# mitschabaude/msm-zprize

Measured on AMD Instinct MI355X. Metric: Mpoint-adds/s (ms per MSM in ms_per_step), higher is better.
Workload: dtype u32 limbs (28-bit lazy Montgomery, i64 accumulate)

## Files before the change

msm_zprize_amd/_native.py:

```python
import ctypes as C
import os

HERE = os.path.dirname(os.path.abspath(__file__))
LIB_PATH = os.environ.get("MSMZ_LIB") or os.path.join(HERE, "libmsmz.so")

MSMZ_N_STAGES = 8
STAGE_NAMES = ["digits", "scan", "scatter", "plan", "accumulate", "reduce", "final", "total"]


class MsmzOpts(C.Structure):
    _fields_ = [("c", C.c_int32), ("glv", C.c_int32), ("safe", C.c_int32), ("buckets", C.c_int32),
                ("timing", C.c_int32), ("reserved", C.c_int32 * 3)]


class MsmzLog(C.Structure):
    _fields_ = [("stage_ms", C.c_float * MSMZ_N_STAGES), ("c", C.c_int32), ("K", C.c_int32), ("rounds", C.c_int32),
                ("glv", C.c_int32), ("n_entries", C.c_uint64), ("n_pairs", C.c_uint64), ("max_bucket", C.c_uint32),
                ("scatter_launches", C.c_uint32), ("scatter_kernel_ms", C.c_float), ("batch_add_ms", C.c_float * 32)]


MSMZ_SRC_DEVICE, MSMZ_SRC_MONTGOMERY, MSMZ_SRC_DEFAULT_STREAM = 1, 2, 4
MSMZ_SRC_COMPRESSED, MSMZ_SRC_SIGN_PARITY = 8, 16
MSMZ_ERR_POINT = 7

# ... 170 lines not shown
    "msmz_scalars_sumcheck_round": (C.c_int, [C.c_void_p, C.POINTER(MsmzSumcheck), C.POINTER(C.c_uint32), C.c_char_p]),
    "msmz_point_add": (C.c_int, [C.c_int, C.c_char_p, C.c_int, C.c_char_p, C.c_int, C.c_char_p, C.POINTER(C.c_int)]),
    "msmz_test_set_glv_bits": (C.c_int, [C.c_void_p, C.c_int]),
    "msmz_test_retries": (C.c_int, [C.c_void_p]),
    "msmz_test_set_limits": (C.c_int, [C.c_void_p, C.c_uint64, C.c_uint64]),
    "msmz_test_passes": (C.c_int, [C.c_void_p, C.POINTER(C.c_uint64), C.POINTER(C.c_uint64)]),
    "msmz_test_scalar_dot_geometry": (None, [C.POINTER(C.c_uint32), C.POINTER(C.c_uint32)]),
    "msmz_test_scalar_scan_geometry": (None, [C.POINTER(C.c_uint32), C.POINTER(C.c_uint32), C.POINTER(C.c_uint32)]),
    "msmz_test_ntt_plan": (C.c_int, [C.c_int, C.c_uint32, C.POINTER(C.c_uint32), C.POINTER(C.c_uint32)]),
    "msmz_test_ntt_geometry": (None, [C.POINTER(C.c_uint32)]),
    "msmz_test_mle_geometry": (None, [C.POINTER(C.c_uint32), C.POINTER(C.c_uint32), C.POINTER(C.c_uint32)]),
    "msmz_test_fixed_base_plan": (C.c_int, [C.c_int, C.c_uint64, C.c_int, C.POINTER(C.c_int32), C.POINTER(C.c_int32),
                                            C.POINTER(C.c_uint64)]),
    "msmz_test_set_fixed_base_window": (C.c_int, [C.c_void_p, C.c_int]),
    "msmz_test_fixed_base_tables": (C.c_int, [C.c_void_p, C.POINTER(C.c_uint64)]),
    "msmz_test_field": (C.c_int, [C.c_void_p, C.c_int, C.c_char_p, C.c_char_p, C.c_uint64, C.c_char_p]),
    "msmz_test_field_limbs": (C.c_int, [C.c_void_p, C.c_int, C.c_void_p, C.c_void_p, C.c_uint64, C.c_void_p,
                                        C.c_char_p]),
    "msmz_test_field_rows": (C.c_int, [C.c_void_p, C.c_int, C.c_void_p, C.c_void_p, C.c_uint64, C.c_uint32, C.c_void_p,
                                       C.c_char_p]),
    "msmz_test_glv": (C.c_int, [C.c_void_p, C.c_char_p, C.c_uint64, C.c_char_p, C.c_char_p, C.c_char_p]),
    "msmz_test_digits": (C.c_int, [C.c_void_p, C.c_char_p, C.c_uint64, C.c_int, C.c_int, C.c_int, C.c_void_p]),
    "msmz_test_sort": (C.c_int, [C.c_void_p, C.c_char_p, C.c_uint64, C.c_int, C.c_int, C.c_int, C.c_void_p, C.c_void_p,
                                 C.c_uint64, C.c_void_p, C.c_uint64]),
    "msmz_test_sort_ex": (C.c_int, [C.c_void_p, C.POINTER(MsmzTestSortArgs)]),
    "msmz_test_point_raw": (C.c_int, [C.c_void_p, C.c_int, C.c_char_p, C.c_char_p, C.c_char_p, C.c_uint64, C.c_int,
                                      C.c_char_p]),
    "msmz_test_point": (C.c_int, [C.c_void_p, C.c_int, C.c_char_p, C.c_char_p, C.c_char_p, C.c_char_p, C.c_uint64,
                                  C.c_char_p]),
    "msmz_test_batch_add": (C.c_int, [C.c_void_p, C.c_int, C.c_int, C.c_char_p, C.c_char_p, C.c_uint64, C.c_char_p,
                                      C.c_char_p, C.c_uint64, C.c_void_p, C.c_uint64, C.c_uint64, C.c_char_p,
                                      C.POINTER(C.c_uint32)]),
    "msmz_test_reduce": (C.c_int, [C.c_void_p, C.POINTER(MsmzTestReduceArgs)]),
    "msmz_test_plan": (C.c_int, [C.c_void_p, C.POINTER(MsmzTestPlanArgs)]),
}

_lib = None


class MsmzError(RuntimeError):
    def __init__(self, status, where):
        self.status = status
        msg = lib().msmz_strerror(status).decode() if _lib is not None else "?"
        super().__init__(f"{where}: msmz status {status} ({msg})")


def lib():
    global _lib
    if _lib is None:
        if not os.path.exists(LIB_PATH):
            raise RuntimeError(f"{LIB_PATH} is missing: run `python -m msm_zprize_amd.build` "
                               "(the MSM has no CPU fallback)")
        l = C.CDLL(LIB_PATH)
        for name, (res, args) in EXPORTS.items():
            fn = getattr(l, name)
            fn.restype = res
            fn.argtypes = args
        _lib = l
    return _lib


def check(status, where):
    if status != 0:
        raise MsmzError(status, where)
```

msm_zprize_amd/csrc/instantiate.h:

```cpp
#pragma once
#include "check_kernels.h"
#include "export_kernels.h"
#include "fixed_kernels.h"
#include "gen_kernels.h"
#include "import_kernels.h"
#include "kernels.h"
#include "mle_kernels.h"
#include "mul_kernels.h"
#include "ntt_kernels.h"
#include "scalar_kernels.h"
#include "scan_kernels.h"
#include "test_kernels.h"

#if !defined(MSMZ_CURVE) || MSMZ_CURVE == 0
#define MSMZ_W0(X) X(Bls377Fp, Bls377Fr)
#else
#define MSMZ_W0(X)
#endif
#if !defined(MSMZ_CURVE) || MSMZ_CURVE == 1
#define MSMZ_W1(X) X(PallasFp, PallasFr)
#else
#define MSMZ_W1(X)
#endif
#if !defined(MSMZ_CURVE) || MSMZ_CURVE == 2
// ... 15 lines not shown
#ifndef MSMZ_BATCH_OCC
#define MSMZ_BATCH_OCC 4
#endif
#ifndef MSMZ_BATCH_BMAX
#define MSMZ_BATCH_BMAX 16
#endif

#define MSMZ_INST_BATCH(F, Fr, PFX)                                                                               \
  PFX template __global__ void k_batch_add<F, MSMZ_BATCH_T, true, MSMZ_BATCH_OCC, MSMZ_BATCH_BMAX>(              \
      uint32_t*, const uint32_t*, const uint2*, uint32_t, uint32_t, int, MsmMeta*);                              \
  PFX template __global__ void k_batch_add<F, MSMZ_BATCH_T, false, MSMZ_BATCH_OCC, MSMZ_BATCH_BMAX>(             \
      uint32_t*, const uint32_t*, const uint2*, uint32_t, uint32_t, int, MsmMeta*);

#define MSMZ_INST_POLICY(P, PFX)                                                                                 \
  PFX template __global__ void k_reduce_quad<P>(uint32_t*, uint32_t*, const uint32_t*, const uint32_t*, uint32_t, \
                                                uint32_t, uint32_t);                                             \
  PFX template __global__ void k_reduce_quad16<P>(uint32_t*, uint32_t*, const uint32_t*, const uint32_t*,        \
                                                  uint32_t, uint32_t, uint32_t);                                 \
  PFX template __global__ void k_reduce_tail<P>(uint32_t*, uint32_t*, uint32_t*, uint32_t*, uint32_t*, uint32_t, \
                                                uint32_t);                                                       \
  PFX template __global__ void k_reduce_rows<P>(uint32_t*, uint32_t*, const uint32_t*, const uint32_t*, uint32_t, \
                                                uint32_t, uint32_t);                                             \
  PFX template __global__ void k_pairsum<P>(uint32_t*, const uint32_t*, uint32_t);                               \
  PFX template __global__ void k_fill_neutral<P>(uint32_t*, uint32_t);                                           \
  PFX template __global__ void k_bucket_sums<P>(uint32_t*, const uint32_t*, const uint32_t*, uint32_t);          \
  PFX template __global__ void k_reduce2d_partial_acc<P>(uint32_t*, const uint32_t*, const uint32_t*, R2Geom, uint32_t); \
  PFX template __global__ void k_pairsum_x4<P>(uint32_t*, const uint32_t*, uint32_t);                            \
  PFX template __global__ void k_bucket_accumulate<P>(uint32_t*, const uint32_t*, const uint32_t*,               \
                                                      const uint32_t*, const uint32_t*, uint32_t, uint32_t, int);

#define MSMZ_INST_REDUCE(F, Fr, PFX)                                                                              \
  PFX template __global__ void k_reduce2d_partial<F>(uint32_t*, const uint32_t*, const uint32_t*, const uint4*,   \
                                                     R2Geom, uint32_t);                                          \
  PFX template __global__ void k_reduce_affine_finish<F>(uint32_t*, uint32_t*, const uint32_t*, const uint32_t*,  \
                                                         const uint2*, const uint4*, F2Geom);                     \
  MSMZ_INST_POLICY(WeierPolicy<F>, PFX)

#define MSMZ_INST_REDUCE_TE(F, Fr, PFX) MSMZ_INST_POLICY(TePolicy<F>, PFX)

#define MSMZ_INST_TEST(F, Fr, P, PFX)                                                                             \
  PFX template __global__ void k_test_field<F>(uint32_t*, const uint32_t*, const uint32_t*, uint32_t, int, uint32_t*); \
  PFX template __global__ void k_test_field_limbs<F>(int32_t*, uint32_t*, const int32_t*, const int32_t*, uint32_t,  \
                                                      int, uint32_t*);                                            \
  PFX template __global__ void k_test_field_rows<F>(int32_t*, uint32_t*, const int32_t*, const int32_t*, uint32_t,   \
                                                     int, uint32_t);                                              \
  PFX template __global__ void k_test_glv<Fr>(uint32_t*, uint32_t*, uint8_t*, const uint32_t*, uint32_t);         \
  PFX template __global__ void k_test_digits<Fr, false>(uint32_t*, const uint32_t*, uint32_t, int, int);          \
  PFX template __global__ void k_test_point<P>(uint32_t*, const uint32_t*, const uint32_t*, const uint8_t*,   \
                                                   const uint8_t*, uint32_t, int);                                \
  PFX template __global__ void k_test_point_raw<P>(uint32_t*, const uint32_t*, const uint32_t*, const uint8_t*, \
                                                       uint32_t, int, int);                                       \
  PFX template __global__ void k_test_accs_in<P>(uint32_t*, const uint32_t*, const uint8_t*, const uint32_t*, \
                                                     uint32_t, uint32_t*);                                        \
  PFX template __global__ void k_test_accs_out<P>(uint32_t*, const uint32_t*, uint32_t);

#define MSMZ_INST_SORT(Fr, PFX, GLV, C, SEG)                                                                      \
  PFX template __global__ void k_hist<Fr, GLV, C, SEG>(uint32_t*, uint16_t*, uint32_t*, MsmMeta*, const uint32_t*, SortGeom, uint32_t, const SegDesc*); \
  PFX template __global__ void k_coarse<Fr, GLV, C, SEG>(uint32_t*, const uint32_t*, const uint32_t*, const uint16_t*, const uint32_t*, SortGeom, uint32_t, const SegDesc*);

#define MSMZ_INST_SCAN(Fr, AM, HB, PFX)                                                                           \
  PFX template __global__ void k_scalars_rec_tile<Fr, AM, HB>(uint32_t*, uint32_t*, const uint32_t*, const uint32_t*, FrConst, uint32_t, uint32_t, uint32_t*); \
  PFX template __global__ void k_scalars_rec_apply<Fr, AM, HB>(uint32_t*, const uint32_t*, const uint32_t*, FrConst, const uint32_t*, uint32_t, uint32_t);

#define MSMZ_INST_SCALAR(Fr, PFX)                                                                                 \
  PFX template __global__ void k_digits<Fr, false>(uint32_t*, uint32_t*, MsmMeta*, const uint32_t*, uint32_t, int, int, int, int); \
  MSMZ_SORT_INSTANCES(MSMZ_INST_SORT, Fr, PFX)                                                                    \
// ... 66 lines not shown
```

msm_zprize_amd/csrc/kernels.h:

```cpp
#pragma once
#include <hip/hip_runtime.h>
#include "constants_gen.h"
#include "plan.h"
#include "curve.h"
#include "fp_rows.h"
#include "scalar.h"

namespace msmz {

constexpr uint32_t REF_NEG = 0x80000000u;
constexpr uint32_t REF_IDX = 0x7fffffffu;

struct MsmMeta {
  uint32_t max_bucket;
  uint32_t n_entries;
  uint32_t error;
  uint32_t rounds;
  uint32_t round_pairs[32];
  uint32_t round_base[32];
};

typedef uint32_t u32x4 __attribute__((ext_vector_type(4)));

#ifndef MSMZ_POINT_PAD
// ... 590 lines not shown
  fe_quad_bcast<0>(PPP, m);
  fe_quad_bcast<1>(Q, m);
  fe_quad_bcast<2>(t, m);
  fe_quad_bcast<3>(u, m);
  fe_pick(r.ZZ, dbl, u, t);
  fe_pick(RR, dbl, t, RR);
  fe_pick(u, dbl, zero, PPP);
  fe_sub(t, RR, u);
  fe_sub(t, t, Q);
  fe_sub(u, t, Q);
  fe_carry(u);
  fe_sub(t, Q, u);
  fe_carry(t);
  fe_sel4(a, s, R, S1, Zc, Zc);
  fe_sel4(m, s, M, p.Y, p.ZZZ, p.ZZZ);
  fe_pick(a, dbl, m, a);
  fe_pick(b, s == 0, t, PPP);
  fe_mul(m, a, b);
  fe_quad_bcast<0>(Q, m);
  fe_quad_bcast<1>(t, m);
  fe_quad_bcast<2>(r.ZZZ, m);
  fe_sub(r.Y, Q, t);
  fe_carry(r.Y);
  r.X = u;
  if (pinf) {
    r = q;
  } else if (qinf) {
    r = p;
  } else if (!dbl && fe_is_zero(P)) {
    if (fe_is_zero(R)) xyzz_dbl(r, p); else xyzz_set_inf(r);
  }
}

template <class F>
__device__ __forceinline__ void te_add_x4(TeExt<F>& r, const TeExt<F>& p, const TeExt<F>& q, int s, bool) {
  Fe<F> a, b, m, A, B, C, D, E, Fv, G, H, t, u, v, w, k;
  fe_sub(t, p.Y, p.X);
  fe_sub(u, q.Y, q.X);
  fe_carry(t);
  fe_carry(u);
  fe_add(v, p.Y, p.X);
  fe_add(w, q.Y, q.X);
  fe_carry(v);
  fe_carry(w);
  fe_sel4(a, s, t, v, p.T, p.Z);
  fe_sel4(b, s, u, w, q.T, q.Z);
  fe_mul(m, a, b);
  fe_quad_bcast<0>(A, m);
  fe_quad_bcast<1>(B, m);
  fe_quad_bcast<2>(t, m);
  fe_quad_bcast<3>(D, m);
  fe_set_const<F>(k, F::K2D);
  fe_mul(C, t, k);
  fe_add(D, D, D);
  fe_sub(E, B, A);
  fe_sub(Fv, D, C);
  fe_add(G, D, C);
  fe_add(H, B, A);
  fe_carry(E);
  fe_carry(Fv);
  fe_carry(G);
  fe_carry(H);
  fe_sel4(a, s, E, G, E, Fv);
  fe_sel4(b, s, Fv, H, H, G);
  fe_mul(m, a, b);
  fe_quad_bcast<0>(r.X, m);
// ... 87 lines not shown
template <class F>
__device__ __forceinline__ void te_add_rows(AccRow<F>& r, const AccRow<F>& p, const AccRow<F>& q, bool,
                                            const RowLane<F>& k) {
  const int s = (int)(__lane_id() >> 4);
  const int32_t pX = p.c[0], pY = p.c[1], pZ = p.c[2], pT = p.c[3];
  const int32_t qX = q.c[0], qY = q.c[1], qZ = q.c[2], qT = q.c[3];
  const int32_t t = fe_carry_row<F>(pY - pX, k), u = fe_carry_row<F>(qY - qX, k);
  const int32_t v = fe_carry_row<F>(pY + pX, k), w = fe_carry_row<F>(qY + qX, k);
  int32_t m = fe_mul_row<F>(row_sel4(s, t, v, pT, pZ), row_sel4(s, u, w, qT, qZ), k);
  const int32_t A = fe_from_row(m, 0), B = fe_from_row(m, 1), TT = fe_from_row(m, 2);
  int32_t D = fe_from_row(m, 3);
  const int32_t C = fe_mul_row<F>(TT, row_const<F>(F::K2D, k.j), k);
  D = D + D;
  const int32_t E = fe_carry_row<F>(B - A, k), Fv = fe_carry_row<F>(D - C, k);
  const int32_t G = fe_carry_row<F>(D + C, k), H = fe_carry_row<F>(B + A, k);
  m = fe_mul_row<F>(row_sel4(s, E, G, E, Fv), row_sel4(s, Fv, H, H, G), k);
  r.c[0] = fe_from_row(m, 0);
  r.c[1] = fe_from_row(m, 1);
  r.c[3] = fe_from_row(m, 2);
  r.c[2] = fe_from_row(m, 3);
}

template <class F_>
struct WeierPolicy : WeierGroup<F_> {
  using G = WeierGroup<F_>;
  using F = F_;
  using typename G::Acc;
  using typename G::Base;
  using G::madd;
  static constexpr int IN_WORDS = PointFmt<F>::STRIDE;
  static constexpr int ACC_WORDS = 4 * F::NW;
  static constexpr int ACC_OCC = 1;
  static __device__ __forceinline__ void add_x4(Acc& r, const Acc& a, const Acc& b, int s, bool dbl) { xyzz_add_x4(r, a, b, s, dbl); }
  using Row = AccRow<F>;
  static __device__ __forceinline__ void add_rows(Row& r, const Row& a, const Row& b, bool dbl, const RowLane<F>& k) { xyzz_add_rows(r, a, b, dbl, k); }
  static __device__ __forceinline__ void identity_row(Row& a, const RowLane<F>& k) { a.c[0] = a.c[1] = k.one; a.c[2] = a.c[3] = 0; }
  static __device__ __forceinline__ void madd(Acc& r, const Acc& a, const uint32_t* rec, uint32_t neg) {
    Affine<F> p;
    bool inf = load_affine<F>(p, rec, neg);
    xyzz_madd(r, a, p, inf);
  }
  static __device__ __forceinline__ void load(Acc& a, const uint32_t* rec) { load_fe4<F>(a.X, a.Y, a.ZZ, a.ZZZ, rec); }
  static __device__ __forceinline__ void store(uint32_t* rec, const Acc& a) { store_fe4<F>(rec, a.X, a.Y, a.ZZ, a.ZZZ); }
  static __device__ __forceinline__ bool load_base(Base& b, const uint32_t* rec) {
    return b.inf = load_affine<F>(b.a, rec, 0);
  }
  static __device__ __forceinline__ bool load_resident_affine(Fe<F>& x, Fe<F>& y, const uint32_t* rec) {
    Affine<F> a;
    const bool inf = load_affine<F>(a, rec, 0);
    x = a.x;
    y = a.y;
    return inf;
  }
  static __device__ __forceinline__ void store_resident(uint32_t* out, uint32_t i, uint32_t n, const Fe<F>& x,
                                                        const Fe<F>& y, bool flagged, int endo) {
    Affine<F> m{x, y};
    store_affine<F>(out + (size_t)i * IN_WORDS, m, flagged);
    if (endo) {
      if (!flagged) {
        Fe<F> beta;
        fe_set_const<F>(beta, F::BETA);
        fe_mul(m.x, x, beta);
      }
      store_affine<F>(out + ((size_t)n + i) * IN_WORDS, m, flagged);
    }
  }
// ... 113 lines not shown
  const uint32_t t = blockIdx.x * blockDim.x + threadIdx.x;
  if (t >= n_chunks) return;
  uint32_t lo = 0, hi = nb;
  while (hi - lo > 1) {
    uint32_t mid = (lo + hi) >> 1;
    if (cscan[mid] <= t) lo = mid; else hi = mid;
  }
  const uint32_t start = off[lo] + ((t - cscan[lo]) << chunk_shift);
  const uint32_t end = min(start + (1u << chunk_shift), off[lo + 1]);
  typename P::Acc acc, tmp;
  P::set_identity(acc);
  for (uint32_t p = start; p < end; p++) {
    const uint32_t rf = refs[p];
    P::madd(tmp, acc, points + (size_t)(rf & REF_IDX) * P::IN_WORDS, rf >> 31);
    acc = tmp;
  }
  P::store(partial + (size_t)t * P::ACC_WORDS, acc);
}

template <class F>
__device__ __forceinline__ void add_bucket(Xyzz<F>& run, uint32_t g, const uint32_t* slots, const uint32_t* points,
                                           const uint4* bfin) {
  const uint4 fin = bfin[g];
  const uint32_t locs[4] = {fin.x, fin.y, fin.z, fin.w};
#pragma unroll 1
  for (int i = 0; i < 4; i++) {
    const uint32_t loc = locs[i];
    if (loc == LOC_NONE) break;
    Affine<F> p;
    const bool inf = load_operand<F, true>(p, loc, slots, points);
    Xyzz<F> tmp;
    xyzz_madd(tmp, run, p, inf);
    run = tmp;
  }
}

template <class P>
__device__ __forceinline__ void quad_fetch(typename P::Acc& got, const typename P::Acc& pub, int src_lane) {
  constexpr int NWORDS = sizeof(typename P::Acc) / 4;
  const int32_t* in = reinterpret_cast<const int32_t*>(&pub);
  int32_t* out = reinterpret_cast<int32_t*>(&got);
#pragma unroll
  for (int j = 0; j < NWORDS; j++) out[j] = __shfl(in[j], src_lane, 64);
}

template <class P>
__global__ void __launch_bounds__(64, MSMZ_REDUCE_OCC) k_reduce_quad(uint32_t* rows_out, uint32_t* c_out, const uint32_t* rows_in,
                                                    const uint32_t* c_in, uint32_t n_in, uint32_t groups,
                                                    uint32_t total) {
  constexpr int XW = P::ACC_WORDS;
  using Acc = typename P::Acc;
  const uint32_t t = blockIdx.x * blockDim.x + threadIdx.x;
  const uint32_t grp = t >> 2, q = t & 3;
  const bool live = grp < total;
  const uint32_t k = live ? grp / groups : 0, A = live ? grp - k * groups : 0;
  const uint32_t e = A * 4 + q;
  const int lane = threadIdx.x & 63, base_lane = lane & ~3;
  Acc r, c, v, w, got;
  P::set_identity(r);
  P::set_identity(c);
  if (live && e < n_in) {
    P::load(r, rows_in + ((size_t)k * n_in + e) * XW);
    P::load(c, c_in + ((size_t)k * n_in + e) * XW);
  }
  {
    const int src[4] = {1, 3, 3, 2};
// ... 187 lines not shown
```

msm_zprize_amd/csrc/msmz.hip:

```cpp
#include "instantiate.h"
namespace msmz {
#define X(F, Fr) MSMZ_INST_BATCH(F, Fr, MSMZ_EXTERN) MSMZ_INST_REDUCE(F, Fr, MSMZ_EXTERN) MSMZ_INST_MISC(F, Fr, MSMZ_EXTERN) MSMZ_INST_GEN(F, Fr, MSMZ_EXTERN) MSMZ_INST_MLE(F, Fr, MSMZ_EXTERN)
MSMZ_WEIERSTRASS_FIELDS(X)
#undef X
#define X(F, Fr) MSMZ_INST_REDUCE_TE(F, Fr, MSMZ_EXTERN) MSMZ_INST_MISC_TE(F, Fr, MSMZ_EXTERN) MSMZ_INST_GEN_TE(F, Fr, MSMZ_EXTERN) MSMZ_INST_MLE(F, Fr, MSMZ_EXTERN)
MSMZ_TE_FIELDS(X)
#undef X
}
#include "test_hooks.h"

namespace msmz {

template <class F_, class Fr_>
struct WeierCfg {
  using F = F_;
  using Fr = Fr_;
  using P = WeierPolicy<F>;
  static constexpr bool TE = false;
  static constexpr bool HAS_ENDO = true;
};

template <class F_, class Fr_>
struct TeCfg {
  using F = F_;
// ... 341 lines not shown
  return c ? c->engine->test_hooks()->test_field_rows(op, a, b, n, live_rows, raw, canon) : MSMZ_ERR_ARG;
}
int msmz_test_glv(msmz_ctx* c, const uint8_t* s, uint64_t n, uint8_t* s0, uint8_t* s1, uint8_t* neg) {
  return c ? c->engine->test_hooks()->test_glv(s, n, s0, s1, neg) : MSMZ_ERR_ARG;
}
int msmz_test_digits(msmz_ctx* c, const uint8_t* s, uint64_t n, int cc, int K, int glv, uint32_t* digits) {
  return c ? c->engine->test_hooks()->test_digits(s, n, cc, K, glv, digits) : MSMZ_ERR_ARG;
}
int msmz_test_sort(msmz_ctx* c, const uint8_t* s, uint64_t n, int cc, int glv, int force_fallback, uint32_t* geom,
                   uint32_t* off, uint64_t off_cap, uint32_t* refs, uint64_t refs_cap) {
  if (!c) return MSMZ_ERR_ARG;
  return c->engine->test_hooks()->test_sort(s, n, cc, glv, force_fallback, geom, off, off_cap, refs, refs_cap);
}
int msmz_test_sort_ex(msmz_ctx* c, const msmz_test_sort_args* a) {
  return c && a ? c->engine->test_hooks()->test_sort_ex(*a) : MSMZ_ERR_ARG;
}
int msmz_test_point_raw(msmz_ctx* c, int op, const uint8_t* a, const uint8_t* b, const uint8_t* neg, uint64_t n, int L,
                        uint8_t* out) {
  return c ? c->engine->test_hooks()->test_point_raw(op, a, b, neg, n, L, out) : MSMZ_ERR_ARG;
}
int msmz_test_point(msmz_ctx* c, int op, const uint8_t* a, const uint8_t* ai, const uint8_t* b, const uint8_t* bi,
                    uint64_t n, uint8_t* out) {
  return c ? c->engine->test_hooks()->test_point(op, a, ai, b, bi, n, out) : MSMZ_ERR_ARG;
}

int msmz_test_batch_add(msmz_ctx* c, int safe, int B, const uint8_t* pxy, const uint8_t* pinf, uint64_t np,
                        const uint8_t* sxy, const uint8_t* sinf, uint64_t ns, const uint32_t* desc, uint64_t n_pairs,
                        uint64_t out_base, uint8_t* out, uint32_t* error) {
  if (!c) return MSMZ_ERR_ARG;
  return c->engine->test_hooks()->test_batch_add(safe, B, pxy, pinf, np, sxy, sinf, ns, desc, n_pairs, out_base, out, error);
}

int msmz_test_reduce(msmz_ctx* c, const msmz_test_reduce_args* a) {
  return c && a ? c->engine->test_hooks()->test_reduce(*a) : MSMZ_ERR_ARG;
}

int msmz_test_plan(msmz_ctx* c, const msmz_test_plan_args* a) {
  return c && a ? c->engine->test_hooks()->test_plan(*a) : MSMZ_ERR_ARG;
}

int msmz_point_add(int curve_id, const uint8_t* a, int ai, const uint8_t* b, int bi, uint8_t* out, int* oi) {
  if (!out || !oi || (!a && !ai) || (!b && !bi)) return MSMZ_ERR_ARG;
  switch (curve_id) {
    case MSMZ_BLS12_377_G1: return host_point_add<CfgBls377::P>(a, ai, b, bi, out, oi);
    case MSMZ_PALLAS: return host_point_add<CfgPallas::P>(a, ai, b, bi, out, oi);
    case MSMZ_BLS12_381_G1: return host_point_add<CfgBls381::P>(a, ai, b, bi, out, oi);
    case MSMZ_ED_ON_BLS12_377: return host_point_add<CfgEd377::P>(a, 0, b, 0, out, oi);
    default: return MSMZ_ERR_UNSUPPORTED;
  }
}

}
```

msm_zprize_amd/csrc/reduce.h:

```cpp
#pragma once
#include <hip/hip_runtime.h>

#include <cstring>

#include "../../include/msmz.h"
#include "batch_add.h"
#include "kernels.h"
#include "plan.h"
#include "store.h"

namespace msmz {

struct ReduceKnobs {
  uint32_t tail_n = (uint32_t)env_int("MSMZ_TAIL_N", REDUCE_TAIL_N);
  uint32_t quad16_max = (uint32_t)env_int("MSMZ_QUAD16", 8192);
  uint32_t pairsum_x4_max = (uint32_t)env_int("MSMZ_PAIRSUM_X4", 16384);
  uint32_t rows_max = (uint32_t)env_int("MSMZ_ROWS_MAX", 512);
};

struct BucketSource {
  const uint32_t* recs;
  const uint32_t* points;
  const uint4* bfin;
  const uint32_t* cscan;

  static BucketSource locations(const uint32_t* slots, const uint32_t* pts, const uint4* bfin) { return {slots, pts, bfin, nullptr}; }
  static BucketSource chunks(const uint32_t* accs, const uint32_t* cscan) { return {accs, nullptr, nullptr, cscan}; }
  static BucketSource per_bucket(const uint32_t* accs) { return {accs, nullptr, nullptr, nullptr}; }
};

template <class Cfg>
class BucketReduce {
  using F = typename Cfg::F;
  using P = typename Cfg::P;
  static constexpr int AW = P::ACC_WORDS;

 public:
  int run_2d(const R2Geom& g, const ReduceKnobs& rk, const BucketSource& src, hipStream_t stream) {
    const uint32_t* lines;
    if (int st = line_sums(g, rk, src, stream, &lines)) return st;
    return weighted_sums(g, rk, stream);
  }

  int line_sums(const R2Geom& g, const ReduceKnobs& rk, const BucketSource& src, hipStream_t stream,
                const uint32_t** lines) {
    const uint32_t n_lines = g.nprob * g.H;
    const uint32_t total = n_lines * g.NC;
    int st;
    if ((st = rows_room(0, total)) || (st = rows_room(1, total))) return st;
    if (src.bfin) {
      if constexpr (!Cfg::TE)
        hipLaunchKernelGGL((k_reduce2d_partial<F>), dim3((total + 127) / 128), dim3(128), 0, stream, rows(0), src.recs,
                           src.points, src.bfin, g, total);
    } else {
      hipLaunchKernelGGL((k_reduce2d_partial_acc<P>), dim3((total + 127) / 128), dim3(128), 0, stream, rows(0), src.recs,
                         src.cscan, g, total);
    }
    cur_ = 0;
    for (uint32_t n = total / 2; n >= n_lines && g.NC > 1; n /= 2) {
      if (n <= rk.pairsum_x4_max) {
        hipLaunchKernelGGL((k_pairsum_x4<P>), dim3((n * 4 + 63) / 64), dim3(64), 0, stream, rows(cur_ ^ 1), rows(cur_), n);
      } else {
        hipLaunchKernelGGL((k_pairsum<P>), dim3((n + 127) / 128), dim3(128), 0, stream, rows(cur_ ^ 1), rows(cur_), n);
      }
      cur_ ^= 1;
      if (n == n_lines) break;
    }
    *lines = rows(cur_);
    return MSMZ_OK;
  }

  int weighted_sums(const R2Geom& g, const ReduceKnobs& rk, hipStream_t stream) {
    const uint32_t n_lines = g.nprob * g.H;
    if (int st = carry_room(cur_, n_lines)) return st;
    hipLaunchKernelGGL((k_fill_neutral<P>), dim3((n_lines + 255) / 256), dim3(256), 0, stream, carry(cur_), n_lines);
    if (int st = levels(rk, g.H, g.nprob, stream)) return st;
    MSMZ_HIP(hipGetLastError());
    return MSMZ_OK;
  }

  int level_inputs(size_t n, uint32_t** rows_out, uint32_t** c_out) {
    int st;
    if ((st = rows_room(0, n)) || (st = carry_room(0, n))) return st;
    cur_ = 0;
    *rows_out = rows(0);
    *c_out = carry(0);
    return MSMZ_OK;
  }

  int levels(const ReduceKnobs& rk, uint32_t n_in, uint32_t nprob, hipStream_t stream) {
    int st;
    const uint32_t rows_max = rk.rows_max < rk.quad16_max ? rk.rows_max : rk.quad16_max;
    while (n_in > rk.tail_n || (n_in > 1 && (uint64_t)nprob * ((n_in + 3) / 4) <= rows_max)) {
      const uint32_t S = 4;
// ... 88 lines not shown
```

msm_zprize_amd/csrc/reduce2d_kernels.h:

```cpp
#pragma once
#include "plan.h"

namespace msmz {

struct R2Chunk {
  uint32_t prob, kw, line, chunk, j0, step, count;
  bool fold;
};
__device__ __forceinline__ R2Chunk r2_chunk(const R2Geom& g, uint32_t t) {
  R2Chunk c;
  const uint32_t per_prob = g.H * g.NC;
  c.prob = t / per_prob;
  const uint32_t u = t - c.prob * per_prob;
  c.kw = c.prob >> 1;
  const bool col = (c.prob & 1u) != 0;
  c.j0 = c.step = c.count = 0;
  if (!col) {
    c.line = u / g.NC;
    c.chunk = u - c.line * g.NC;
    c.j0 = c.line * g.D + c.chunk;
    c.step = g.NC;
    c.count = g.chr;
  } else if (u < g.D * g.NC) {
    c.chunk = u / g.D;
// ... 10 lines not shown
  return c;
}

template <class P>
__device__ __forceinline__ void add_accs(typename P::Acc& acc, const uint32_t* accs, uint32_t q0, uint32_t q1) {
  typename P::Acc tmp, p;
  for (uint32_t q = q0; q < q1; q++) {
    P::load(p, accs + (size_t)q * P::ACC_WORDS);
    P::add(tmp, acc, p);
    acc = tmp;
  }
}

template <class F>
__global__ void __launch_bounds__(128, MSMZ_REDUCE_OCC) k_reduce2d_partial(uint32_t* part, const uint32_t* slots,
                                                                           const uint32_t* points, const uint4* bfin,
                                                                           R2Geom g, uint32_t total) {
  const uint32_t t = blockIdx.x * blockDim.x + threadIdx.x;
  if (t >= total) return;
  const R2Chunk c = r2_chunk(g, t);
  Xyzz<F> acc;
  xyzz_set_inf(acc);
#pragma unroll 1
  for (uint32_t i = 0; i < c.count; i++) {
    const uint32_t j = c.j0 + i * c.step;
    if (j >= 1) add_bucket<F>(acc, c.kw * g.L + (j - 1), slots, points, bfin);
  }
  if (c.fold) {
    for (int twice = 0; twice < 2; twice++) add_bucket<F>(acc, c.kw * g.L + (g.L - 1), slots, points, bfin);
  }
  WeierPolicy<F>::store(part + ((size_t)(c.prob * g.H + c.line) * g.NC + c.chunk) * 4 * F::NW, acc);
}

template <class P>
__global__ void __launch_bounds__(128, MSMZ_REDUCE_OCC) k_reduce2d_partial_acc(uint32_t* part, const uint32_t* accs,
                                                                               const uint32_t* cscan, R2Geom g,
                                                                               uint32_t total) {
  const uint32_t t = blockIdx.x * blockDim.x + threadIdx.x;
  if (t >= total) return;
  const R2Chunk c = r2_chunk(g, t);
  typename P::Acc acc;
  P::set_identity(acc);
  auto range = [&](uint32_t j, uint32_t& a, uint32_t& b) {
    a = b = 0;
    if (j >= 1) {
      const size_t gb = (size_t)c.kw * g.L + (j - 1);
      a = cscan ? cscan[gb] : (uint32_t)gb;
      b = cscan ? cscan[gb + 1] : (uint32_t)gb + 1u;
    }
  };
  uint32_t qa = 0, qb = 0;
  if (c.count) range(c.j0, qa, qb);
#pragma unroll 1
  for (uint32_t i = 0; i < c.count; i++) {
    uint32_t na = 0, nb = 0;
    if (i + 1 < c.count) range(c.j0 + (i + 1) * c.step, na, nb);
    add_accs<P>(acc, accs, qa, qb);
    qa = na;
    qb = nb;
  }
  if (c.fold) {
    range(g.L, qa, qb);
    for (int twice = 0; twice < 2; twice++) add_accs<P>(acc, accs, qa, qb);
  }
  P::store(part + ((size_t)(c.prob * g.H + c.line) * g.NC + c.chunk) * P::ACC_WORDS, acc);
}
// ... 9 lines not shown
  const uint32_t q0 = cscan[gb], q1 = cscan[gb + 1];
  if (q1 > q0) {
    P::load(acc, accs + (size_t)q0 * XW);
    for (uint32_t q = q0 + 1; q < q1; q++) {
      P::load(p, accs + (size_t)q * XW);
      P::add(tmp, acc, p);
      acc = tmp;
    }
  }
  P::store(out + (size_t)gb * XW, acc);
}

template <class P>
__global__ void __launch_bounds__(256) k_fill_neutral(uint32_t* out, uint32_t n) {
  const uint32_t t = blockIdx.x * blockDim.x + threadIdx.x;
  if (t >= n) return;
  typename P::Acc z;
  P::set_identity(z);
  P::store(out + (size_t)t * P::ACC_WORDS, z);
}

template <class P>
__global__ void __launch_bounds__(128, MSMZ_REDUCE_OCC) k_pairsum(uint32_t* out, const uint32_t* in, uint32_t n_out) {
  constexpr int XW = P::ACC_WORDS;
  const uint32_t t = blockIdx.x * blockDim.x + threadIdx.x;
  if (t >= n_out) return;
  typename P::Acc a, b, r;
  P::load(a, in + (size_t)(2 * t) * XW);
  P::load(b, in + (size_t)(2 * t + 1) * XW);
  P::add(r, a, b);
  P::store(out + (size_t)t * XW, r);
}

template <class P>
__global__ void __launch_bounds__(64, MSMZ_Q16_OCC) k_pairsum_x4(uint32_t* out, const uint32_t* in, uint32_t n_out) {
  constexpr int XW = P::ACC_WORDS;
  const uint32_t t = blockIdx.x * blockDim.x + threadIdx.x;
  const uint32_t i = t >> 2;
  const int s = (int)(t & 3);
  const bool live = i < n_out;
  typename P::Acc a, b, r;
  P::set_identity(a);
  P::set_identity(b);
  if (live) {
    P::load(a, in + (size_t)(2 * i) * XW);
    P::load(b, in + (size_t)(2 * i + 1) * XW);
  }
  P::add_x4(r, a, b, s, false);
  if (live && s == 0) P::store(out + (size_t)i * XW, r);
}

}
```

Before: 4712.

## Split XYZZ bucket-reduce partial and pairsum across lane pairs with DPP exchange

```diff
diff --git a/msm_zprize_amd/_native.py b/msm_zprize_amd/_native.py
--- a/msm_zprize_amd/_native.py
+++ b/msm_zprize_amd/_native.py
@@ -226,6 +226,7 @@
                                       C.c_char_p, C.c_uint64, C.c_void_p, C.c_uint64, C.c_uint64, C.c_char_p,
                                       C.POINTER(C.c_uint32)]),
     "msmz_test_reduce": (C.c_int, [C.c_void_p, C.POINTER(MsmzTestReduceArgs)]),
+    "msmz_test_reduce_forms": (C.c_int, [C.c_void_p, C.POINTER(MsmzTestReduceArgs), C.c_int32, C.c_uint32]),
     "msmz_test_plan": (C.c_int, [C.c_void_p, C.POINTER(MsmzTestPlanArgs)]),
 }
 
diff --git a/msm_zprize_amd/csrc/instantiate.h b/msm_zprize_amd/csrc/instantiate.h
--- a/msm_zprize_amd/csrc/instantiate.h
+++ b/msm_zprize_amd/csrc/instantiate.h
@@ -71,6 +71,9 @@
 #define MSMZ_INST_REDUCE(F, Fr, PFX)                                                                              \
   PFX template __global__ void k_reduce2d_partial<F>(uint32_t*, const uint32_t*, const uint32_t*, const uint4*,   \
                                                      R2Geom, uint32_t);                                          \
+  PFX template __global__ void k_reduce2d_partial_x2<F>(uint32_t*, const uint32_t*, const uint32_t*, const uint4*, \
+                                                        R2Geom, uint32_t);                                       \
+  PFX template __global__ void k_pairsum_x2<WeierPolicy<F>>(uint32_t*, const uint32_t*, uint32_t);                \
   PFX template __global__ void k_reduce_affine_finish<F>(uint32_t*, uint32_t*, const uint32_t*, const uint32_t*,  \
                                                          const uint2*, const uint4*, F2Geom);                     \
   MSMZ_INST_POLICY(WeierPolicy<F>, PFX)
diff --git a/msm_zprize_amd/csrc/kernels.h b/msm_zprize_amd/csrc/kernels.h
--- a/msm_zprize_amd/csrc/kernels.h
+++ b/msm_zprize_amd/csrc/kernels.h
@@ -646,6 +646,225 @@
   }
 }
 
+constexpr int PAIR_SWAP = 0xB1;
+constexpr int PAIR_A = 0xA0;
+constexpr int PAIR_B = 0xF5;
+template <int CTRL, class F>
+__device__ __forceinline__ void fe_pair(Fe<F>& r, const Fe<F>& a) {
+#pragma unroll
+  for (int j = 0; j < F::N; j++) r.l[j] = __builtin_amdgcn_update_dpp(0, a.l[j], CTRL, 0xf, 0xf, false);
+}
+template <int CTRL>
+__device__ __forceinline__ uint32_t word_pair(uint32_t v) {
+  return (uint32_t)__builtin_amdgcn_update_dpp(0, (int)v, CTRL, 0xf, 0xf, false);
+}
+template <int CTRL>
+__device__ __forceinline__ bool flag_pair(bool v) {
+  return word_pair<CTRL>(v ? 1u : 0u) != 0;
+}
+
+template <class F>
+struct XyzzHalf {
+  Fe<F> X, W, ZZZ;
+};
+template <class F>
+struct XyzzPair {
+  Fe<F> U, Z;
+};
+
+template <class F>
+__device__ __forceinline__ void xyzz_set_inf_x2(XyzzHalf<F>& r, bool lb) {
+  Fe<F> one, zero;
+  fe_set_const<F>(one, F::ONE);
+  fe_zero(zero);
+  r.X = one;
+  fe_pick(r.W, lb, one, zero);
+  r.ZZZ = zero;
+}
+
+template <class F>
+__device__ __forceinline__ void xyzz_half_from_pair(XyzzHalf<F>& r, const XyzzPair<F>& p, bool lb) {
+  Fe<F> xu, xz;
+  fe_pair<PAIR_SWAP>(xu, p.U);
+  fe_pair<PAIR_SWAP>(xz, p.Z);
+  fe_pick(r.X, lb, xu, p.U);
+  fe_pick(r.W, lb, p.U, p.Z);
+  fe_pick(r.ZZZ, lb, p.Z, xz);
+}
+
+template <bool MIXED, class F>
+__device__ __forceinline__ void xyzz_dbl_x2(XyzzHalf<F>& r, const Fe<F>& c, const Fe<F>& z, bool lb) {
+  Fe<F> U, a, b, m, XX, V, M, MM, W, yw, S, t, x3;
+  fe_add(U, c, c);
+  fe_carry(U);
+  fe_pick(a, lb, U, c);
+  fe_sqr(m, a);
+  fe_pair<PAIR_A>(XX, m);
+  fe_pair<PAIR_B>(V, m);
+  fe_add(M, XX, XX);
+  fe_add(M, M, XX);
+  fe_carry(M);
+  fe_pick(a, lb, U, M);
+  fe_pick(b, lb, V, M);
+  fe_mul(m, a, b);
+  fe_pair<PAIR_A>(MM, m);
+  fe_pair<PAIR_B>(W, m);
+  fe_pick(b, lb, W, V);
+  fe_mul(yw, c, b);
+  fe_pair<PAIR_A>(S, yw);
+  fe_sub(t, MM, S);
+  fe_sub(x3, t, S);
+  fe_sub(t, S, x3);
+  fe_carry(t);
+  fe_mul(m, M, t);
+  fe_sub(t, m, yw);
+  fe_carry(t);
+  fe_carry(x3);
+  r.X = x3;
+  if constexpr (MIXED) {
+    fe_pick(r.W, lb, t, V);
+    r.ZZZ = W;
+  } else {
+    fe_pick(b, lb, W, V);
+    fe_mul(m, b, z);
+    fe_pick(r.W, lb, t, m);
+    fe_pair<PAIR_B>(r.ZZZ, m);
+  }
+}
+
+template <class F>
+__device__ __forceinline__ void xyzz_madd_x2(XyzzHalf<F>& r, const Fe<F>& c, bool rec_inf, bool lb) {
+  if (rec_inf) return;
+  if (flag_pair<PAIR_A>(fe_is_zero(r.W))) {
+    Fe<F> one;
+    fe_set_const<F>(one, F::ONE);
+    fe_pair<PAIR_A>(r.X, c);
+    fe_pick(r.W, lb, c, one);
+    r.ZZZ = one;
+    return;
+  }
+  Fe<F> a, b, m, d, PP, RR, PPP, Q, t, u, m4;
+  fe_pick(b, lb, r.ZZZ, r.W);
+  fe_mul(m, c, b);
+  fe_pick(a, lb, r.W, r.X);
+  fe_sub(d, m, a);
+  fe_carry(d);
+  const bool dz = fe_is_zero(d);
+  if (flag_pair<PAIR_A>(dz)) {
+    if (flag_pair<PAIR_B>(dz)) xyzz_dbl_x2<true>(r, c, c, lb); else xyzz_set_inf_x2(r, lb);
+    return;
+  }
+  fe_sqr(m, d);
+  fe_pair<PAIR_A>(PP, m);
+  fe_pair<PAIR_B>(RR, m);
+  fe_pick(a, lb, r.X, d);
+  fe_mul(m, a, PP);
+  fe_pair<PAIR_A>(PPP, m);
+  fe_pair<PAIR_B>(Q, m);
+  fe_sub(t, RR, PPP);
+  fe_sub(t, t, Q);
+  fe_sub(u, t, Q);
+  fe_carry(u);
+  fe_sub(t, Q, u);
+  fe_carry(t);
+  fe_pick(b, lb, PPP, PP);
+  fe_mul(m4, r.W, b);
+  fe_pick(a, lb, d, r.ZZZ);
+  fe_pick(b, lb, t, PPP);
+  fe_mul(m, a, b);
+  fe_sub(t, m, m4);
+  fe_carry(t);
+  r.X = u;
+  fe_pick(r.W, lb, t, m4);
+  fe_pair<PAIR_A>(r.ZZZ, m);
+}
+
+template <class F>
+__device__ __forceinline__ void xyzz_add_x2(XyzzHalf<F>& r, const XyzzPair<F>& p, const XyzzPair<F>& q, bool lb) {
+  if (flag_pair<PAIR_A>(fe_is_zero(p.Z))) {
+    xyzz_half_from_pair(r, q, lb);
+    return;
+  }
+  if (flag_pair<PAIR_A>(fe_is_zero(q.Z))) {
+    xyzz_half_from_pair(r, p, lb);
+    return;
+  }
+  Fe<F> a, b, m, m1, d, PP, RR, U1, PPP, Q, t, u, zz, m6;
+  fe_mul(m1, p.U, q.Z);
+  fe_mul(m, q.U, p.Z);
+  fe_sub(d, m, m1);
+  const bool dz = fe_is_zero(d);
+  if (flag_pair<PAIR_A>(dz)) {
+    if (flag_pair<PAIR_B>(dz)) xyzz_dbl_x2<false>(r, p.U, p.Z, lb); else xyzz_set_inf_x2(r, lb);
+    return;
+  }
+  fe_sqr(m, d);
+  fe_pair<PAIR_A>(PP, m);
+  fe_pair<PAIR_B>(RR, m);
+  fe_pair<PAIR_A>(U1, m1);
+  fe_pick(a, lb, U1, d);
+  fe_mul(m, a, PP);
+  fe_pair<PAIR_A>(PPP, m);
+  fe_pair<PAIR_B>(Q, m);
+  fe_sub(t, RR, PPP);
+  fe_sub(t, t, Q);
+  fe_sub(u, t, Q);
+  fe_carry(u);
+  fe_sub(t, Q, u);
+  fe_carry(t);
+  fe_mul(zz, p.Z, q.Z);
+  fe_pick(a, lb, m1, zz);
+  fe_pick(b, lb, PPP, PP);
+  fe_mul(m6, a, b);
+  fe_pair<PAIR_B>(m, zz);
+  fe_pick(a, lb, d, m);
+  fe_pick(b, lb, t, PPP);
+  fe_mul(m, a, b);
+  fe_sub(t, m, m6);
+  fe_carry(t);
+  r.X = u;
+  fe_pick(r.W, lb, t, m6);
+  fe_pair<PAIR_A>(r.ZZZ, m);
+}
+
+template <class F>
+__device__ __forceinline__ void fe_load_vec(Fe<F>& a, const uint32_t* src) {
+  const u32x4* s4 = reinterpret_cast<const u32x4*>(src);
+  uint32_t w[F::NW];
+#pragma unroll
+  for (int i = 0; i < F::NW / 4; i++) {
+    const u32x4 v = s4[i];
+    w[4 * i] = v.x;
+    w[4 * i + 1] = v.y;
+    w[4 * i + 2] = v.z;
+    w[4 * i + 3] = v.w;
+  }
+  fe_unpack<F>(a, w);
+}
+template <class F>
+__device__ __forceinline__ void fe_store_vec(uint32_t* dst, const Fe<F>& a) {
+  uint32_t w[F::NW];
+  fe_store<F>(w, a);
+  u32x4* d4 = reinterpret_cast<u32x4*>(dst);
+#pragma unroll
+  for (int i = 0; i < F::NW / 4; i++) d4[i] = u32x4{w[4 * i], w[4 * i + 1], w[4 * i + 2], w[4 * i + 3]};
+}
+template <class F>
+__device__ __forceinline__ void xyzz_load_pair(XyzzPair<F>& p, const uint32_t* rec, bool lb) {
+  rec += lb ? F::NW : 0;
+  fe_load_vec<F>(p.U, rec);
+  fe_load_vec<F>(p.Z, rec + 2 * F::NW);
+}
+template <class F>
+__device__ __forceinline__ void xyzz_store_half(uint32_t* rec, const XyzzHalf<F>& a, bool lb) {
+  Fe<F> t;
+  rec += lb ? F::NW : 0;
+  fe_pick(t, lb, a.W, a.X);
+  fe_store_vec<F>(rec, t);
+  fe_pick(t, lb, a.ZZZ, a.W);
+  fe_store_vec<F>(rec + 2 * F::NW, t);
+}
+
 template <class F>
 __device__ __forceinline__ void te_add_x4(TeExt<F>& r, const TeExt<F>& p, const TeExt<F>& q, int s, bool) {
   Fe<F> a, b, m, A, B, C, D, E, Fv, G, H, t, u, v, w, k;
@@ -799,6 +1018,11 @@
   static constexpr int ACC_WORDS = 4 * F::NW;
   static constexpr int ACC_OCC = 1;
   static __device__ __forceinline__ void add_x4(Acc& r, const Acc& a, const Acc& b, int s, bool dbl) { xyzz_add_x4(r, a, b, s, dbl); }
+  using AccPair = XyzzPair<F>;
+  using AccHalf = XyzzHalf<F>;
+  static __device__ __forceinline__ void load_pair(AccPair& a, const uint32_t* rec, bool lb) { xyzz_load_pair<F>(a, rec, lb); }
+  static __device__ __forceinline__ void add_x2(AccHalf& r, const AccPair& a, const AccPair& b, bool lb) { xyzz_add_x2(r, a, b, lb); }
+  static __device__ __forceinline__ void store_half(uint32_t* rec, const AccHalf& a, bool lb) { xyzz_store_half<F>(rec, a, lb); }
   using Row = AccRow<F>;
   static __device__ __forceinline__ void add_rows(Row& r, const Row& a, const Row& b, bool dbl, const RowLane<F>& k) { xyzz_add_rows(r, a, b, dbl, k); }
   static __device__ __forceinline__ void identity_row(Row& a, const RowLane<F>& k) { a.c[0] = a.c[1] = k.one; a.c[2] = a.c[3] = 0; }
@@ -978,6 +1202,52 @@
     Xyzz<F> tmp;
     xyzz_madd(tmp, run, p, inf);
     run = tmp;
+  }
+}
+
+template <class F>
+__device__ __forceinline__ uint32_t load_operand_half(Fe<F>& c, uint32_t loc, const uint32_t* slots, const uint32_t* points,
+                                                      bool lb) {
+  if constexpr (SlotFmt<F>::PACKED) {
+    int cs;
+    uint32_t neg;
+    const u32x4* s4 = reinterpret_cast<const u32x4*>(operand_address<F>(loc, slots, points, cs, neg)) +
+                      (lb ? F::NW / 4 : 0) * cs;
+    uint32_t w[F::NW];
+    uint32_t o = 0;
+#pragma unroll
+    for (int i = 0; i < F::NW / 4; i++) {
+      const u32x4 v = s4[i * cs];
+      w[4 * i] = v.x;
+      w[4 * i + 1] = v.y;
+      w[4 * i + 2] = v.z;
+      w[4 * i + 3] = v.w;
+      o |= v.x | v.y | v.z | v.w;
+    }
+    Fe<F> v;
+    fe_unpack<F>(v, w);
+    fe_cneg(c, v, lb ? neg : 0u);
+    return o;
+  } else {
+    Affine<F> p;
+    const bool inf = load_operand<F, true>(p, loc, slots, points);
+    fe_pick(c, lb, p.y, p.x);
+    return inf ? 0u : 1u;
+  }
+}
+
+template <class F>
+__device__ __forceinline__ void add_bucket_x2(XyzzHalf<F>& run, uint32_t g, const uint32_t* slots, const uint32_t* points,
+                                              const uint4* bfin, bool lb) {
+  const uint4 fin = bfin[g];
+  const uint32_t locs[4] = {fin.x, fin.y, fin.z, fin.w};
+#pragma unroll 1
+  for (int i = 0; i < 4; i++) {
+    const uint32_t loc = locs[i];
+    if (loc == LOC_NONE) break;
+    Fe<F> c;
+    const uint32_t o = load_operand_half<F>(c, loc, slots, points, lb);
+    xyzz_madd_x2(run, c, (o | word_pair<PAIR_SWAP>(o)) == 0, lb);
   }
 }
 
diff --git a/msm_zprize_amd/csrc/msmz.hip b/msm_zprize_amd/csrc/msmz.hip
--- a/msm_zprize_amd/csrc/msmz.hip
+++ b/msm_zprize_amd/csrc/msmz.hip
@@ -397,7 +397,10 @@
 }
 
 int msmz_test_reduce(msmz_ctx* c, const msmz_test_reduce_args* a) {
-  return c && a ? c->engine->test_hooks()->test_reduce(*a) : MSMZ_ERR_ARG;
+  return c && a ? c->engine->test_hooks()->test_reduce(*a, 0, 0) : MSMZ_ERR_ARG;
+}
+int msmz_test_reduce_forms(msmz_ctx* c, const msmz_test_reduce_args* a, int32_t partial_form, uint32_t pairsum_x2_max) {
+  return c && a ? c->engine->test_hooks()->test_reduce(*a, partial_form, pairsum_x2_max) : MSMZ_ERR_ARG;
 }
 
 int msmz_test_plan(msmz_ctx* c, const msmz_test_plan_args* a) {
diff --git a/msm_zprize_amd/csrc/reduce.h b/msm_zprize_amd/csrc/reduce.h
--- a/msm_zprize_amd/csrc/reduce.h
+++ b/msm_zprize_amd/csrc/reduce.h
@@ -16,6 +16,8 @@
   uint32_t quad16_max = (uint32_t)env_int("MSMZ_QUAD16", 8192);
   uint32_t pairsum_x4_max = (uint32_t)env_int("MSMZ_PAIRSUM_X4", 16384);
   uint32_t rows_max = (uint32_t)env_int("MSMZ_ROWS_MAX", 512);
+  uint32_t partial_x2 = (uint32_t)env_int("MSMZ_PARTIAL_X2", 1);
+  uint32_t pairsum_x2_max = (uint32_t)env_int("MSMZ_PAIRSUM_X2", 1u << 30);
 };
 
 struct BucketSource {
@@ -49,9 +51,14 @@
     int st;
     if ((st = rows_room(0, total)) || (st = rows_room(1, total))) return st;
     if (src.bfin) {
-      if constexpr (!Cfg::TE)
-        hipLaunchKernelGGL((k_reduce2d_partial<F>), dim3((total + 127) / 128), dim3(128), 0, stream, rows(0), src.recs,
-                           src.points, src.bfin, g, total);
+      if constexpr (!Cfg::TE) {
+        if (rk.partial_x2)
+          hipLaunchKernelGGL((k_reduce2d_partial_x2<F>), dim3((uint32_t)(((uint64_t)total * 2 + 127) / 128)), dim3(128), 0,
+                             stream, rows(0), src.recs, src.points, src.bfin, g, total);
+        else
+          hipLaunchKernelGGL((k_reduce2d_partial<F>), dim3((total + 127) / 128), dim3(128), 0, stream, rows(0), src.recs,
+                             src.points, src.bfin, g, total);
+      }
     } else {
       hipLaunchKernelGGL((k_reduce2d_partial_acc<P>), dim3((total + 127) / 128), dim3(128), 0, stream, rows(0), src.recs,
                          src.cscan, g, total);
@@ -60,6 +67,10 @@
     for (uint32_t n = total / 2; n >= n_lines && g.NC > 1; n /= 2) {
       if (n <= rk.pairsum_x4_max) {
         hipLaunchKernelGGL((k_pairsum_x4<P>), dim3((n * 4 + 63) / 64), dim3(64), 0, stream, rows(cur_ ^ 1), rows(cur_), n);
+      } else if (!Cfg::TE && n <= rk.pairsum_x2_max) {
+        if constexpr (!Cfg::TE)
+          hipLaunchKernelGGL((k_pairsum_x2<P>), dim3((uint32_t)(((uint64_t)n * 2 + 127) / 128)), dim3(128), 0, stream,
+                             rows(cur_ ^ 1), rows(cur_), n);
       } else {
         hipLaunchKernelGGL((k_pairsum<P>), dim3((n + 127) / 128), dim3(128), 0, stream, rows(cur_ ^ 1), rows(cur_), n);
       }
diff --git a/msm_zprize_amd/csrc/reduce2d_kernels.h b/msm_zprize_amd/csrc/reduce2d_kernels.h
--- a/msm_zprize_amd/csrc/reduce2d_kernels.h
+++ b/msm_zprize_amd/csrc/reduce2d_kernels.h
@@ -66,6 +66,30 @@
   WeierPolicy<F>::store(part + ((size_t)(c.prob * g.H + c.line) * g.NC + c.chunk) * 4 * F::NW, acc);
 }
 
+#ifndef MSMZ_PARTIAL_X2_OCC
+#define MSMZ_PARTIAL_X2_OCC 3
+#endif
+template <class F>
+__global__ void __launch_bounds__(128, MSMZ_PARTIAL_X2_OCC) k_reduce2d_partial_x2(uint32_t* part, const uint32_t* slots,
+                                                                                  const uint32_t* points, const uint4* bfin,
+                                                                                  R2Geom g, uint32_t total) {
+  const uint32_t t = blockIdx.x * blockDim.x + threadIdx.x;
+  if ((t >> 1) >= total) return;
+  const bool lb = (t & 1u) != 0;
+  const R2Chunk c = r2_chunk(g, t >> 1);
+  XyzzHalf<F> acc;
+  xyzz_set_inf_x2(acc, lb);
+#pragma unroll 1
+  for (uint32_t i = 0; i < c.count; i++) {
+    const uint32_t j = c.j0 + i * c.step;
+    if (j >= 1) add_bucket_x2<F>(acc, c.kw * g.L + (j - 1), slots, points, bfin, lb);
+  }
+  if (c.fold) {
+    for (int twice = 0; twice < 2; twice++) add_bucket_x2<F>(acc, c.kw * g.L + (g.L - 1), slots, points, bfin, lb);
+  }
+  xyzz_store_half<F>(part + ((size_t)(c.prob * g.H + c.line) * g.NC + c.chunk) * 4 * F::NW, acc, lb);
+}
+
 template <class P>
 __global__ void __launch_bounds__(128, MSMZ_REDUCE_OCC) k_reduce2d_partial_acc(uint32_t* part, const uint32_t* accs,
                                                                                const uint32_t* cscan, R2Geom g,
@@ -141,6 +165,24 @@
   P::store(out + (size_t)t * XW, r);
 }
 
+#ifndef MSMZ_PAIRSUM_X2_OCC
+#define MSMZ_PAIRSUM_X2_OCC 3
+#endif
+template <class P>
+__global__ void __launch_bounds__(128, MSMZ_PAIRSUM_X2_OCC) k_pairsum_x2(uint32_t* out, const uint32_t* in, uint32_t n_out) {
+  constexpr int XW = P::ACC_WORDS;
+  const uint32_t t = blockIdx.x * blockDim.x + threadIdx.x;
+  const uint32_t i = t >> 1;
+  if (i >= n_out) return;
+  const bool lb = (t & 1u) != 0;
+  typename P::AccPair a, b;
+  typename P::AccHalf r;
+  P::load_pair(a, in + (size_t)(2 * i) * XW, lb);
+  P::load_pair(b, in + (size_t)(2 * i + 1) * XW, lb);
+  P::add_x2(r, a, b, lb);
+  P::store_half(out + (size_t)i * XW, r, lb);
+}
+
 template <class P>
 __global__ void __launch_bounds__(64, MSMZ_Q16_OCC) k_pairsum_x4(uint32_t* out, const uint32_t* in, uint32_t n_out) {
   constexpr int XW = P::ACC_WORDS;
```

Result: no change. 4779, median of 6 (+1.4%).
